# BuTTerK3ks/AA-RMVSNet

Measured on AMD Instinct MI355X. Metric: depth-hypotheses/sec (ref-views x H x W x D / s), higher is better.
Workload: dtype fp32-class split-fp16 (3 products: cells, deconvs, omega conv on f16 MFMA, lo*lo dropped, fp32 accumulate; fp32 elsewhere); 1 GPU; dtu_eval_1600x1184_n7_d512; ref_views_per_gpu=1, views=7, H=1184, W=1600, D=512, global_batch=1, parallelism=ref-view shard x1

## Files before the change

### aa-rmvsnet_amd/csrc/warp_cost.hip

```cpp
#include <hip/hip_runtime.h>

#include <cfloat>
#include <climits>
#include <cstdlib>
#include <cstring>

#include "device_common.h"

namespace aarmvs {

__device__ __forceinline__ void sample_pos(const float* __restrict__ m, float depth, float x,
                                           float y, int H, int W, float& ix, float& iy) {
  float p[3];
#pragma unroll
  for (int k = 0; k < 3; ++k) {
    const float rx = __fadd_rn(__fadd_rn(__fmul_rn(m[4 * k + 0], x), __fmul_rn(m[4 * k + 1], y)),
                               m[4 * k + 2]);
    p[k] = __fadd_rn(__fmul_rn(rx, depth), m[4 * k + 3]);
  }
  float z = p[2];
  if (z == 0.0f) z = __fadd_rn(z, 1e-4f);
  const float px = __fdiv_rn(p[0], z), py = __fdiv_rn(p[1], z);
  const float gx = __fsub_rn(__fdiv_rn(px, (float)(W - 1) * 0.5f), 1.0f);
  const float gy = __fsub_rn(__fdiv_rn(py, (float)(H - 1) * 0.5f), 1.0f);
// ... 677 lines not shown

typedef _Float16 half8 __attribute__((ext_vector_type(8)));
typedef _Float16 half4 __attribute__((ext_vector_type(4)));
typedef _Float16 half2_t __attribute__((ext_vector_type(2)));
typedef float float2_t __attribute__((ext_vector_type(2)));
typedef float floatx4 __attribute__((ext_vector_type(4)));
typedef float floatx16 __attribute__((ext_vector_type(16)));

typedef __attribute__((address_space(3))) void* lds_void_ptr;
__device__ __forceinline__ void dma16(__amdgpu_buffer_rsrc_t r, float* wave_dst, uint32_t off,
                                      uint32_t soff = 0) {
  __builtin_amdgcn_raw_ptr_buffer_load_lds(r, (lds_void_ptr)wave_dst, 16, off, soff, 0, 0);
}
__device__ __forceinline__ uint32_t split_pair(float a, float b, uint32_t& lo_bits) {
  const uint32_t hb = __builtin_bit_cast(uint32_t, __builtin_convertvector((float2_t){a, b}, half2_t));
  float la, lb;
  asm("v_fma_mix_f32 %0, %1, -1.0, %2 op_sel_hi:[1,0,0]" : "=v"(la) : "v"(hb), "v"(a));
  asm("v_fma_mix_f32 %0, %1, -1.0, %2 op_sel:[1,0,0] op_sel_hi:[1,0,0]" : "=v"(lb) : "v"(hb), "v"(b));
  lo_bits = __builtin_bit_cast(uint32_t, __builtin_convertvector((float2_t){la, lb}, half2_t));
  return hb;
}
__device__ __forceinline__ void dma_wait() {
  __builtin_amdgcn_s_waitcnt(0x0F70);
}


constexpr int kMTileH = 16;
template <int TW>
struct OmegaTile {
  static constexpr int NT = kMTileH * TW;
  static constexpr int OUTH = kMTileH - 2, OUTW = TW - 2;
  static constexpr int BOXPX = 2 * NT;
  static int tiles(int H, int W) { return ((W + OUTW - 1) / OUTW) * ((H + OUTH - 1) / OUTH); }
  __device__ static int tiles_d(int H, int W) { return ((W + OUTW - 1) / OUTW) * ((H + OUTH - 1) / OUTH); }
};
#ifndef AARMVS_OMEGA_TW
#define AARMVS_OMEGA_TW 16
#endif
constexpr int kOmegaTW = AARMVS_OMEGA_TW;

template <int CTRL, int ROWS>
__device__ __forceinline__ double dpp_f64_u(double v) {
  const long long b = __double_as_longlong(v);
  const int lo = __builtin_amdgcn_mov_dpp((int)(b & 0xffffffffll), CTRL, ROWS, 0xF, false);
  const int hi = __builtin_amdgcn_mov_dpp((int)(b >> 32), CTRL, ROWS, 0xF, false);
  return __longlong_as_double(((long long)hi << 32) | (unsigned)lo);
}
__device__ __forceinline__ void wave_sum2_d(double& u, double& w) {
  u += dpp_f64_u<0xB1, 0xF>(u);
  w += dpp_f64_u<0xB1, 0xF>(w);
  u += dpp_f64_u<0x4E, 0xF>(u);
  w += dpp_f64_u<0x4E, 0xF>(w);
  u += dpp_f64_u<0x141, 0xF>(u);
  w += dpp_f64_u<0x141, 0xF>(w);
  u += dpp_f64_u<0x140, 0xF>(u);
  w += dpp_f64_u<0x140, 0xF>(w);
  u += dpp_f64_u<0x142, 0xA>(u);
  w += dpp_f64_u<0x142, 0xA>(w);
  u += dpp_f64_u<0x143, 0xC>(u);
  w += dpp_f64_u<0x143, 0xC>(w);
  auto rl = [](double v) {
    const long long b = __double_as_longlong(v);
    const int lo = __builtin_amdgcn_readlane((int)(b & 0xffffffffll), 63);
    const int hi = __builtin_amdgcn_readlane((int)(b >> 32), 63);
    return __longlong_as_double(((long long)hi << 32) | (unsigned)lo);
  };
  u = rl(u);
  w = rl(w);
}

struct OmegaPos {
  int tile, ty, tx, v, kp;
};
template <int NW>
__device__ __forceinline__ void omega_block_sum(const double (*ws)[2], double& s0, double& s1) {
  s0 = 0.0;
  s1 = 0.0;
  for (int w = 0; w < NW; ++w) {
    s0 += ws[w][0];
    s1 += ws[w][1];
  }
}

template <int ABL, int TW, bool BAL, typename PA>
__device__ __forceinline__ void omega_item(PA& a, const float* __restrict__ P,
                                           const float* __restrict__ Rel,
                                           const unsigned* __restrict__ xbound, const OmegaPos ip,
                                           double (*wsum)[OmegaTile<TW>::NT / 64][2], int par,
                                           bool has_prev, const OmegaPos pv) {
  using T = OmegaTile<TW>;
  constexpr int kMThreads = T::NT, kMBoxPx = T::BOXPX, kMOutH = T::OUTH, kMOutW = T::OUTW;
  constexpr int NB = (2 * kMBoxPx + kMThreads - 1) / kMThreads;
  static_assert(TW == 16 || TW == 32, "the row sums shift by DPP along one haloed row");
  constexpr int kRefFl = (kMBoxPx + 1) * 8;
  constexpr int YFL = kRefFl + 2 * kMThreads * 4;
  static_assert(2 * kMThreads * 4 <= YFL, "the row-sum images fit in the box space");
  __shared__ __attribute__((aligned(16))) float smem[YFL];
  float* const box = smem;
  float4* const zms = reinterpret_cast<float4*>(smem);
  float4* const zps = zms + kMThreads;
  __shared__ int red[kMThreads / 64][4];
  int tid;
  asm volatile("v_mov_b32 %0, %1" : "=v"(tid) : "v"((int)threadIdx.x));
  const int lane = tid & 63, wave = tid >> 6;
  const int b = blockIdx.z;
  const int H = a.H, W = a.W, HW = H * W, nsrc = a.nsrc;
  const int v = ip.v, kp = ip.kp;
  const int y0 = ip.ty * kMOutH, x0 = ip.tx * kMOutW;
  const int hy = tid / TW, hx = tid % TW;
  const int gy = y0 - 1 + hy, gx = x0 - 1 + hx;
  const bool in_img = gy >= 0 && gy < H && gx >= 0 && gx < W;
  const bool interior = in_img && hy >= 1 && hy <= kMOutH && hx >= 1 && hx <= kMOutW;
  float* const rimg = smem + kRefFl;

  const float dep = a.dvals[b * a.D + a.d_next + kp];
  const float* __restrict__ m = Rel + 12 * (v * a.B + b);
  const uint32_t fbytes = (uint32_t)((size_t)kC * HW * 4);
  const uint32_t cbytes = (uint32_t)HW * 32u;
  const __amdgpu_buffer_rsrc_t rref = uniform_rsrc(a.ref + (size_t)b * kC * HW, fbytes);
  const __amdgpu_buffer_rsrc_t rsrc = uniform_rsrc(a.src[v] + (size_t)b * kC * HW, fbytes);
  TapF tf{};
  int lx = INT_MAX, ly = INT_MAX, bhx = INT_MIN, bhy = INT_MIN;
  if (in_img) {
    if constexpr ((ABL & 16) != 0) {
      tf.xf = (float)gx + 0.25f * dep * 1e-3f;
      tf.yf = (float)gy;
      tf.wt[0] = tf.wt[1] = tf.wt[2] = tf.wt[3] = 0.25f;
      tf.xf = floorf(tf.xf);
    } else {
      tf = tap_f(m, dep, gx, gy, H, W);
    }
    box_extend(tf, H, W, lx, ly, bhx, bhy);
  }
  const Box bx = box_reduce<kMThreads / 64>(lx, ly, bhx, bhy, red);
  if (tid < 8) box[kMBoxPx * 8 + tid] = 0.f;
  if (has_prev && tid == 0) {
    double s0, s1;
    omega_block_sum<kMThreads / 64>(wsum[par ^ 1], s0, s1);
    if (!(ABL & 64)) part_put(a, pv.kp, b, pv.v, pv.tile, s0, s1);
  }
  const bool lds = bx.nx * bx.ny <= min(kMBoxPx, a.box_cap);
  const uint32_t zp = lds ? (uint32_t)kMBoxPx : fbytes / 32u;
  TapP tp = tap_p4(tf, in_img, H, W, lds, bx, zp);
  const int items = lds ? bx.nx * bx.ny * 2 : 0;
  const uint32_t mg = box_magic(bx.nx);
  uint32_t boff[NB];
#pragma unroll
  for (int j = 0; j < NB; ++j) {
    const int i = tid + j * kMThreads, p = i >> 1, r = box_row(p, bx.nx, mg);
    const uint32_t gp = __umul24((uint32_t)(bx.y0 + r), (uint32_t)W) + (uint32_t)bx.x0 +
                        ((uint32_t)p - __umul24((uint32_t)r, (uint32_t)bx.nx));
    boff[j] = gp * 32u + 16u * (uint32_t)img_half((uint32_t)p, i & 1);
  }
  const uint32_t rpix = in_img ? (uint32_t)(gy * W + gx) * 32u : fbytes;
  const int wave_s = __builtin_amdgcn_readfirstlane(wave);
  auto stage = [&](int c) {
    const uint32_t cb = (uint32_t)c * cbytes;
#pragma unroll
    for (int j = 0; j < NB; ++j)
      if (!(ABL & 2) && tid + j * kMThreads < items)
        dma16(rsrc, box + (j * kMThreads + wave_s * 64) * 4, boff[j], cb);
    if (!(ABL & 8)) {
      dma16(rref, rimg + (wave_s * 64) * 4, rpix, cb);
      dma16(rref, rimg + (kMThreads + wave_s * 64) * 4, rpix + 16u, cb);
    }
  };
  int e = 0;
  {
    const float bound = __uint_as_float(*xbound);
    if (bound > 0.0f) {
      const int k = ilogbf(bound);
      e = k >= 134 ? 120 : (k < -100 ? -114 : k - 14);
      e += e & 1;
    }
  }
  const float dsc = ldexpf(1.0f, -(e / 2));
#pragma unroll
  for (int k = 0; k < 4; ++k) tp.wt[k] = __fmul_rn(tp.wt[k], dsc);
  const float* __restrict__ w0t = P + a.off_ow0t;
  const half8* __restrict__ owm = reinterpret_cast<const half8*>(P + a.off_owm);
  floatx16 acc0, acc1;
  if constexpr ((ABL & 1) != 0) {
#pragma unroll
    for (int r = 0; r < 16; ++r) acc0[r] = acc1[r] = 0.f;
  }
  float o4[4] = {0.f, 0.f, 0.f, 0.f};

  stage(0);
  dma_wait();
  __syncthreads();
#pragma unroll 1
  for (int c = 0; c < 4; ++c) {
    const float* const bx_c = box;
    float4 g0, g1;
    if (ABL & 4) {
      g0 = g1 = make_float4(tp.wt[0], tp.wt[1], tp.wt[2], tp.wt[3]);
    } else if (lds) {
      g0 = bil4(img_ld(bx_c, tp.pix[0], 0), img_ld(bx_c, tp.pix[1], 0), img_ld(bx_c, tp.pix[2], 0),
                img_ld(bx_c, tp.pix[3], 0), tp);
      g1 = bil4(img_ld(bx_c, tp.pix[0], 1), img_ld(bx_c, tp.pix[1], 1), img_ld(bx_c, tp.pix[2], 1),
                img_ld(bx_c, tp.pix[3], 1), tp);
    } else {
      g0 = bil4(ld_c8(rsrc, tp.pix[0], 2 * c, HW), ld_c8(rsrc, tp.pix[1], 2 * c, HW),
                ld_c8(rsrc, tp.pix[2], 2 * c, HW), ld_c8(rsrc, tp.pix[3], 2 * c, HW), tp);
      g1 = bil4(ld_c8(rsrc, tp.pix[0], 2 * c + 1, HW), ld_c8(rsrc, tp.pix[1], 2 * c + 1, HW),
                ld_c8(rsrc, tp.pix[2], 2 * c + 1, HW), ld_c8(rsrc, tp.pix[3], 2 * c + 1, HW), tp);
    }
    const float4 rf0 = *reinterpret_cast<const float4*>(rimg + tid * 4);
    const float4 rf1 = *reinterpret_cast<const float4*>(rimg + (kMThreads + tid) * 4);
    auto dsq = [&](float g, float r) {
      const float dd = __fmaf_rn(r, -dsc, g);
      return __fmul_rn(dd, dd);
    };
    const float sq[8] = {dsq(g0.x, rf0.x), dsq(g0.y, rf0.y), dsq(g0.z, rf0.z), dsq(g0.w, rf0.w),
                         dsq(g1.x, rf1.x), dsq(g1.y, rf1.y), dsq(g1.z, rf1.z), dsq(g1.w, rf1.w)};
    half8 Bd, Bl, Bl2;
    if constexpr ((ABL & 128) == 0) {
      Bd = owm[(c * 3 + 0) * 64 + lane];
      Bl = owm[(c * 3 + 1) * 64 + lane];
      Bl2 = owm[(c * 3 + 2) * 64 + lane];
    }
    __syncthreads();
    if (c < 3) stage(c + 1);
    {
      const float* wt = w0t + (4 * kC + 8 * c) * 4;
#pragma unroll
      for (int j = 0; j < 8; ++j)
#pragma unroll
        for (int co = 0; co < 4; ++co) o4[co] = fmaf(sq[j], wt[j * 4 + co], o4[co]);
    }
    uint32_t hw[4], lw[4];
#pragma unroll
    for (int i = 0; i < 4; ++i) hw[i] = split_pair(sq[2 * i], sq[2 * i + 1], lw[i]);
#pragma unroll
    for (int i = 0; i < 4; ++i) {
      const auto r = __builtin_amdgcn_permlane32_swap(hw[i], lw[i], false, false);
      hw[i] = r[0];
      lw[i] = r[1];
    }
    if (BAL && (c & 1)) {
#pragma unroll
      for (int i = 0; i < 4; ++i) {
        hw[i] ^= 0x80008000u;
        lw[i] ^= 0x80008000u;
      }
    }
    if (BAL && c > 0) {
#pragma unroll
      for (int r = 0; r < 16; ++r) {
        acc0[r] = -acc0[r];
        acc1[r] = -acc1[r];
      }
    }
    const half8 A0 = __builtin_bit_cast(half8, u32x4{hw[0], hw[1], hw[2], hw[3]});
    const half8 A1 = __builtin_bit_cast(half8, u32x4{lw[0], lw[1], lw[2], lw[3]});
    if constexpr ((ABL & 128) != 0) {
      Bd = A1;
      Bl = A0;
      Bl2 = A1;
    }
    if (!(ABL & 1)) {
      if (c == 0) {
        const floatx16 z = {};
        acc0 = __builtin_amdgcn_mfma_f32_32x32x16_f16(Bd, A0, z, 0, 0, 0);
        acc1 = __builtin_amdgcn_mfma_f32_32x32x16_f16(Bd, A1, z, 0, 0, 0);
      } else {
        acc0 = __builtin_amdgcn_mfma_f32_32x32x16_f16(Bd, A0, acc0, 0, 0, 0);
        acc1 = __builtin_amdgcn_mfma_f32_32x32x16_f16(Bd, A1, acc1, 0, 0, 0);
      }
      acc0 = __builtin_amdgcn_mfma_f32_32x32x16_f16(Bl, A0, acc0, 0, 0, 0);
      acc1 = __builtin_amdgcn_mfma_f32_32x32x16_f16(Bl, A1, acc1, 0, 0, 0);
      acc0 = __builtin_amdgcn_mfma_f32_32x32x16_f16(Bl2, A0, acc0, 0, 0, 0);
      acc1 = __builtin_amdgcn_mfma_f32_32x32x16_f16(Bl2, A1, acc1, 0, 0, 0);
    } else {
      acc0[0] += (float)A0[0] + (float)Bd[1];
      acc1[0] += (float)A1[0] + (float)Bl[1];
    }
    if (c < 3) {
      dma_wait();
      __syncthreads();
    }
  }
  static constexpr int kShr = TW == 16 ? 0x111 : 0x138, kShl = TW == 16 ? 0x101 : 0x130;
  auto shr1 = [](float x) {
    return __int_as_float(__builtin_amdgcn_update_dpp(0, __float_as_int(x), kShr, 0xF, 0xF, true));
  };
  auto shl1 = [](float x) {
    return __int_as_float(__builtin_amdgcn_update_dpp(0, __float_as_int(x), kShl, 0xF, 0xF, true));
  };
  float zmr[4], zpr[4], z0[4];
#pragma unroll
  for (int co = 0; co < 4; ++co) {
    const float r0 = (shr1(acc0[co]) + acc0[4 + co]) + shl1(acc0[8 + co]);
    const float r1 = (shr1(acc1[co]) + acc1[4 + co]) + shl1(acc1[8 + co]);
    const auto zz = __builtin_amdgcn_permlane32_swap(__float_as_uint(r0), __float_as_uint(r1), false, false);
    zmr[co] = __uint_as_float(zz[0]);
    zpr[co] = __uint_as_float(zz[1]);
    const auto t35 = __builtin_amdgcn_permlane32_swap(__float_as_uint(acc0[12 + co]),
                                                      __float_as_uint(acc1[12 + co]), false, false);
    z0[co] = shr1(__uint_as_float(t35[0])) + shl1(__uint_as_float(t35[1]));
  }
  if constexpr ((ABL & 32) == 0) {
    zms[tid] = make_float4(zmr[0], zmr[1], zmr[2], zmr[3]);
    zps[tid] = make_float4(zpr[0], zpr[1], zpr[2], zpr[3]);
  }
  __syncthreads();
  double ps = 0.0, pss = 0.0;
  if (interior) {
    float g4[4];
    if constexpr ((ABL & 32) != 0) {
#pragma unroll
      for (int co = 0; co < 4; ++co) g4[co] = (zmr[co] + z0[co]) + zpr[co];
    } else {
      const float4 up = zms[tid - TW], dn = zps[tid + TW];
      g4[0] = (up.x + z0[0]) + dn.x;
      g4[1] = (up.y + z0[1]) + dn.y;
      g4[2] = (up.z + z0[2]) + dn.z;
      g4[3] = (up.w + z0[3]) + dn.w;
    }
    if (BAL) {
#pragma unroll
      for (int co = 0; co < 4; ++co) g4[co] = -g4[co];
    }
    const float pe = ldexpf(1.0f, e);
    const float isc = P[a.off_owm_scale] * pe;
    const float* __restrict__ b0 = P + a.off_ob0;
    float4 out;
    out.x = fmaf(g4[0], isc, o4[0] * pe) + b0[0];
    out.y = fmaf(g4[1], isc, o4[1] * pe) + b0[1];
    out.z = fmaf(g4[2], isc, o4[2] * pe) + b0[2];
    out.w = fmaf(g4[3], isc, o4[3] * pe) + b0[3];
    a.t1_next[kp * a.t1_kstride + ((size_t)b * nsrc + v) * HW + gy * W + gx] = out;
    ps = ((double)out.x + (double)out.y) + ((double)out.z + (double)out.w);
    pss = ((double)out.x * out.x + (double)out.y * out.y) + ((double)out.z * out.z + (double)out.w * out.w);
  }
  wave_sum2_d(ps, pss);
  if (lane == 0) {
    wsum[par][wave][0] = ps;
    wsum[par][wave][1] = pss;
  }
}

#ifndef AARMVS_OMEGA_WAVES
#define AARMVS_OMEGA_WAVES 4
#endif
template <int ABL = 0, int TW = kOmegaTW, bool BAL = false>
__global__ void __launch_bounds__(OmegaTile<TW>::NT) __attribute__((amdgpu_waves_per_eu(AARMVS_OMEGA_WAVES)))
omega_mfma_kernel(PipeArgs a, const float* __restrict__ P, const float* __restrict__ Rel,
                  const unsigned* __restrict__ xbound) {
  if (blockDim.x != OmegaTile<TW>::NT) return;
  const int ipb = a.omega_ipb > 1 ? a.omega_ipb : 1;
  const int npl = a.npl, nsrc = a.nsrc;
  const int tiles_x = (a.W + OmegaTile<TW>::OUTW - 1) / OmegaTile<TW>::OUTW;
  const int total = OmegaTile<TW>::tiles_d(a.H, a.W) * nsrc * npl;
  const int seq0 = xcd_tile(blockIdx.x, gridDim.x) * ipb;
  OmegaPos ip;
  ip.tile = seq0 / (nsrc * npl);
  {
    const int vk = seq0 - ip.tile * (nsrc * npl);
    ip.v = vk / npl;
    ip.kp = vk - ip.v * npl;
    ip.ty = ip.tile / tiles_x;
    ip.tx = ip.tile - ip.ty * tiles_x;
  }
  constexpr int NW = OmegaTile<TW>::NT / 64;
  __shared__ double wsum[2][NW][2];
  OmegaPos pv = ip;
  int it = 0;
#pragma unroll 1
  for (; it < ipb; ++it) {
    if (seq0 + it >= total) break;
    if (it) {
      pv = ip;
      if (++ip.kp == npl) {
        ip.kp = 0;
        if (++ip.v == nsrc) {
          ip.v = 0;
          ++ip.tile;
          if (++ip.tx == tiles_x) {
            ip.tx = 0;
            ++ip.ty;
          }
        }
      }
    }
    uint32_t z;
    asm volatile("s_mov_b32 %0, 0" : "=s"(z));
    typedef const __attribute__((address_space(4))) PipeArgs KPipeArgs;
    KPipeArgs& ka = *(KPipeArgs*)((const __attribute__((address_space(4))) char*)&a + z);
    omega_item<ABL, TW, BAL>(ka, P, Rel, xbound, ip, wsum, it & 1, it > 0, pv);
  }
  if (it > 0) {
    __syncthreads();
    if (threadIdx.x == 0) {
      double s0, s1;
      omega_block_sum<NW>(wsum[(it - 1) & 1], s0, s1);
      if (!(ABL & 64)) part_put(a, ip.kp, (int)blockIdx.z, ip.v, ip.tile, s0, s1);
    }
  }
}

template <int STAGE>
__global__ void __launch_bounds__(256) omega_stats_kernel(PipeArgs a,
                                                          const float* __restrict__ P) {
  __shared__ double red[2 * 4];
  __shared__ GnStat gs[2];
  const int v = blockIdx.y, b = blockIdx.z / a.npl, kp = blockIdx.z - b * a.npl;
  const int HW = a.H * a.W;
  double* const st = a.st_next + kp * a.st_kstride;
  if (threadIdx.x < STAGE)
    gs[threadIdx.x] = stat_read(st + st_index(b, v, threadIdx.x, a.nsrc), 4.0 * HW);
  __syncthreads();
  OmegaP o;
  load_omega(a, P, o);
  const float4* t1 = a.t1_next + kp * a.t1_kstride + ((size_t)b * a.nsrc + v) * HW;
  double part[2] = {0.0, 0.0};
  const int gstride = gridDim.x * blockDim.x;
  for (int p0 = blockIdx.x * blockDim.x + threadIdx.x; p0 < HW; p0 += 4 * gstride) {
    float4 qs[4];
#pragma unroll
    for (int u = 0; u < 4; ++u) {
      const int p = p0 + u * gstride;
      qs[u] = p < HW ? t1[p] : make_float4(0.f, 0.f, 0.f, 0.f);
    }
#pragma unroll
    for (int u = 0; u < 4; ++u) {
    if (p0 + u * gstride >= HW) break;
    const float4 q = qs[u];
    const float t[4] = {q.x, q.y, q.z, q.w};
    float aa[4], t2[4];
    gn_relu4(t, gs[0], o.g0w, o.g0b, true, aa);
    conv1x1_4(aa, o.w1, o.b1, t2);
    float r[4];
    if constexpr (STAGE == 1) {
#pragma unroll
      for (int c = 0; c < 4; ++c) r[c] = t2[c];
    } else {
      float bb[4];
      gn_relu4(t2, gs[1], o.g1w, o.g1b, true, bb);
      conv1x1_4(bb, o.w2, o.b2, r);
    }
    part[0] += ((double)r[0] + (double)r[1]) + ((double)r[2] + (double)r[3]);
    part[1] += ((double)r[0] * r[0] + (double)r[1] * r[1]) + ((double)r[2] * r[2] + (double)r[3] * r[3]);
    }
  }
  block_sum_d<2>(part, red);
  if (threadIdx.x == 0) part_put(a, kp, b, v, blockIdx.x, part[0], part[1]);
}

__global__ void __launch_bounds__(256) stat_reduce_kernel(PipeArgs a, int stage) {
  __shared__ double red[2][256];
  const int g = blockIdx.x, v = g % a.nsrc, b = (g / a.nsrc) % a.B, kp = g / (a.nsrc * a.B);
  const double* pp = a.part + 2 * (size_t)g * a.part_n;
  double s = 0.0, ss = 0.0;
  for (int i = threadIdx.x; i < a.part_n; i += 256) {
    s += pp[2 * i];
    ss += pp[2 * i + 1];
  }
  red[0][threadIdx.x] = s;
  red[1][threadIdx.x] = ss;
  __syncthreads();
  for (int o = 128; o > 0; o >>= 1) {
    if (threadIdx.x < o) {
      red[0][threadIdx.x] += red[0][threadIdx.x + o];
      red[1][threadIdx.x] += red[1][threadIdx.x + o];
    }
    __syncthreads();
  }
  if (threadIdx.x == 0) {
    double* st = a.st_next + kp * a.st_kstride + st_index(b, v, stage, a.nsrc);
    st[0] = red[0][0];
    st[1] = red[1][0];
  }
}

static PipeArgs pipe_args(const CostArgs& ca, const SweepGeom& g, const Workspace& ws) {
  const ParamLayout& L = param_layout();
  PipeArgs a{};
  a.ref = ca.ref;
  for (int v = 0; v < AARMVS_MAX_SRC; ++v) a.src[v] = v < g.nsrc ? ca.src[v] : nullptr;
  a.rel = ca.rel;
  a.dvals = ca.depth_values;
  a.D = g.D;
  a.params = ca.params;
  a.x = ws.x;
  a.B = g.B;
  a.H = g.H;
  a.W = g.W;
  a.nsrc = g.nsrc;
  a.box_cap = INT_MAX;
  a.npl = 1;
  a.omega_k = 0;
  a.off_ow0 = L.pk_off[P_OW0];
  a.off_ow0t = L.ow0t_off;
  a.off_owb_scale = L.owb_scale_off;
  a.off_owm = L.owm_off;
  a.off_owm_scale = L.owb_scale_off;
  a.off_ob0 = L.pk_off[P_OB0];
  a.off_og0w = L.pk_off[P_OG0W];
  a.off_og0b = L.pk_off[P_OG0B];
  a.off_ow1 = L.pk_off[P_OW1];
  a.off_ob1 = L.pk_off[P_OB1];
  a.off_og1w = L.pk_off[P_OG1W];
  a.off_og1b = L.pk_off[P_OG1B];
  a.off_ow2 = L.pk_off[P_OW2];
  a.off_ob2 = L.pk_off[P_OB2];
  a.off_og2w = L.pk_off[P_OG2W];
  a.off_og2b = L.pk_off[P_OG2B];
  a.off_owo = L.pk_off[P_OWO];
  a.off_obo = L.pk_off[P_OBO];
  return a;
}

static int pipe_box_cap() {
  const char* s = std::getenv("AARMVS_PIPE_BOX_CAP");
  return (s && *s) ? std::max(4, std::atoi(s)) : INT_MAX;
}

static int omega_ipb(int items, int cu_count) {
  const char* s = std::getenv("AARMVS_OMEGA_IPB");
  if (s && *s) return std::max(1, std::min(8, std::atoi(s)));
  int ipb = 8;
  while (ipb > 1 && (items + ipb - 1) / ipb < 8 * std::max(1, cu_count)) ipb >>= 1;
  return ipb;
}

constexpr int kCostXPlanes = 2;
static int cost_x_planes() {
  const char* s = std::getenv("AARMVS_COST_X_PLANES");
  const int v = (s && *s) ? std::atoi(s) : kCostXPlanes;
  return v >= 4 ? 4 : v >= 2 ? 2 : 1;
}

static PipeArgs pipe_args_c8(const CostArgs& ca, const SweepGeom& g, const Workspace& ws) {
  PipeArgs a = pipe_args(ca, g, ws);
  a.ref = ws.feat8[0];
  for (int v = 0; v < g.nsrc; ++v) a.src[v] = ws.feat8[1 + v];
  a.box_cap = pipe_box_cap();
  return a;
}

static void group_strides(PipeArgs& a, const Workspace& ws, int n) {
  a.npl = n;
  a.t1_kstride = ws.t1_plane;
  a.st_kstride = ws.omega_stats_bytes / sizeof(double);
  a.x_kstride = ws.x_plane;
}

hipError_t launch_cost_x_group(const CostArgs& ca, const SweepGeom& g, const Workspace& ws, int d0,
                               int n, float* x0, float* omega_out, int omega_k, hipStream_t s) {
  PipeArgs a = pipe_args_c8(ca, g, ws);
  group_strides(a, ws, n);
  a.d_prev = d0;
  a.d_next = -1;
  a.x = x0;
  a.t1_prev = reinterpret_cast<const float4*>(ws.t1);
  a.st_prev = ws.omega_stats;
  a.omega_out = omega_out;
  a.omega_k = omega_out ? omega_k : -1;
  const int ntiles = ((g.W + kTileW - 1) / kTileW) * ((g.H + kXRows - 1) / kXRows);
  const int pp = cost_x_planes();
  const dim3 grid(ntiles * ((n + pp - 1) / pp), g.B), block(2 * kXRows * kTileW);
  ProfScope ps(s, K_COST_X);
  if (pp == 4)
    hipLaunchKernelGGL((cost_x_planes_kernel<kXRows, 4>), grid, block, 0, s, a, a.params, a.rel);
  else if (pp == 2)
    hipLaunchKernelGGL((cost_x_planes_kernel<kXRows, 2>), grid, block, 0, s, a, a.params, a.rel);
  else
    hipLaunchKernelGGL(cost_x_kernel<2>, grid, block, 0, s, a, a.params, a.rel);
  return hipGetLastError();
}

hipError_t launch_omega_group(const CostArgs& ca, const SweepGeom& g, const Workspace& ws, int d0,
                              int n, hipStream_t s, bool balanced) {
  PipeArgs a = pipe_args_c8(ca, g, ws);
  group_strides(a, ws, n);
  a.d_prev = -1;
  a.d_next = d0;
  a.t1_next = reinterpret_cast<float4*>(ws.t1);
  a.st_next = ws.omega_stats;
  a.part = ws.omega_part;
  hipError_t e;
  const int nred = n * g.B * g.nsrc;
  if ((e = hipMemsetAsync(ws.omega_stats, 0, (size_t)n * ws.omega_stats_bytes, s)) != hipSuccess)
    return e;
  {
    const int ntiles = OmegaTile<kOmegaTW>::tiles(g.H, g.W);
    ProfScope ps(s, K_OMEGA_CONV);
    a.part_n = ntiles;
    a.omega_ipb = omega_ipb(ntiles * g.nsrc * n * g.B, g.cu_count);
    const int nblk = (ntiles * g.nsrc * n + a.omega_ipb - 1) / a.omega_ipb;
    if (balanced)
      hipLaunchKernelGGL((omega_mfma_kernel<0, kOmegaTW, true>), dim3(nblk, 1, g.B),
                         dim3(OmegaTile<kOmegaTW>::NT), 0, s, a, a.params, a.rel, ws.xbound);
    else
      hipLaunchKernelGGL((omega_mfma_kernel<0, kOmegaTW>), dim3(nblk, 1, g.B),
                         dim3(OmegaTile<kOmegaTW>::NT), 0, s, a, a.params, a.rel, ws.xbound);
    if ((e = hipGetLastError()) != hipSuccess) return e;
  }
  {
    ProfScope ps(s, K_STAT_REDUCE);
    hipLaunchKernelGGL(stat_reduce_kernel, dim3(nred), dim3(256), 0, s, a, 0);
  }
  if ((e = hipGetLastError()) != hipSuccess) return e;
  const int HW = g.H * g.W;
  const int pblk =
      std::max(1, std::min((HW + 1023) / 1024, 8 * g.cu_count / std::max(1, g.B * g.nsrc) + 1));
  a.part_n = pblk;
  {
    ProfScope ps(s, K_OMEGA1);
    hipLaunchKernelGGL(omega_stats_kernel<1>, dim3(pblk, g.nsrc, g.B * n), dim3(256), 0, s, a,
                       a.params);
  }
  if ((e = hipGetLastError()) != hipSuccess) return e;
  {
    ProfScope ps(s, K_STAT_REDUCE);
    hipLaunchKernelGGL(stat_reduce_kernel, dim3(nred), dim3(256), 0, s, a, 1);
  }
  if ((e = hipGetLastError()) != hipSuccess) return e;
  {
    ProfScope ps(s, K_OMEGA2);
    hipLaunchKernelGGL(omega_stats_kernel<2>, dim3(pblk, g.nsrc, g.B * n), dim3(256), 0, s, a,
                       a.params);
  }
  if ((e = hipGetLastError()) != hipSuccess) return e;
  {
    ProfScope ps(s, K_STAT_REDUCE);
    hipLaunchKernelGGL(stat_reduce_kernel, dim3(nred), dim3(256), 0, s, a, 2);
  }
  return hipGetLastError();
}

__global__ void __launch_bounds__(256) nchw_to_c8_kernel(const float* __restrict__ src,
                                                         float* __restrict__ dst, int HW,
                                                         unsigned* __restrict__ xbound) {
  __shared__ float t[kC][65];
  __shared__ float wmax[4];
  const int b = blockIdx.y, p0 = blockIdx.x * 64;
  const float* s = src + (size_t)b * kC * HW;
  float4* d = reinterpret_cast<float4*>(dst + (size_t)b * kC * HW);
  const int px = threadIdx.x & 63;
  float mx = 0.f;
#pragma unroll
  for (int j = 0; j < 8; ++j) {
    const int c = (threadIdx.x >> 6) + 4 * j;
    const float v = p0 + px < HW ? s[(size_t)c * HW + p0 + px] : 0.f;
    t[c][px] = v;
    const float av = fabsf(v);
    mx = (av > mx || av != av) ? av : mx;
  }
  if (xbound) {
#pragma unroll
    for (int o = 32; o > 0; o >>= 1) {
      const float q = __shfl_xor(mx, o, 64);
      mx = (q > mx || q != q) ? q : mx;
    }
    if ((threadIdx.x & 63) == 0) wmax[threadIdx.x >> 6] = mx;
  }
  __syncthreads();
  if (xbound && threadIdx.x == 0) {
    float m = 0.f;
    for (int w = 0; w < 4; ++w) m = (wmax[w] > m || wmax[w] != wmax[w]) ? wmax[w] : m;
    const float bound = 8.0f * m * m;
    const unsigned bits = __float_as_uint(bound != bound ? INFINITY : bound);
    if (bits > __hip_atomic_load(xbound, __ATOMIC_RELAXED, __HIP_MEMORY_SCOPE_AGENT))
      atomicMax(xbound, bits);
  }
#pragma unroll
  for (int j = 0; j < 2; ++j) {
    const int idx = threadIdx.x + 256 * j, ch = idx >> 7, q = (idx & 127) >> 1, h = idx & 1;
    const int c0 = 8 * ch + 4 * h;
    if (p0 + q < HW)
      d[((size_t)ch * HW + p0 + q) * 2 + h] =
          make_float4(t[c0][q], t[c0 + 1][q], t[c0 + 2][q], t[c0 + 3][q]);
  }
}
// ... 897 lines not shown
```

Measured before the change: 1.230 billion depth-hypotheses/s.

## Process two depth planes per omega item sharing one staged source box

The omega MFMA kernel can now handle a pair of adjacent depth planes in one item. Both planes' taps are folded into one shared LDS source box, so the staged box, the reference image reads and the weight fragments are loaded once and serve two planes of MFMA accumulation. If the combined box does not fit in LDS, the kernel falls back to single-plane items. This is meant to cut the repeated DMA staging and synchronisation per plane, at the cost of more live registers (waves_per_eu is lowered to 3) and more complex control flow. It is enabled by default when there are multiple planes per group and the unbalanced path is in use.

Result: faster. 1.260 billion depth-hypotheses/s (median of 6 runs) (+2.5%).

```diff
diff --git a/aa-rmvsnet_amd/csrc/warp_cost.hip b/aa-rmvsnet_amd/csrc/warp_cost.hip
--- a/aa-rmvsnet_amd/csrc/warp_cost.hip
+++ b/aa-rmvsnet_amd/csrc/warp_cost.hip
@@ -783,24 +783,31 @@
   }
 }
 
-template <int ABL, int TW, bool BAL, typename PA>
-__device__ __forceinline__ void omega_item(PA& a, const float* __restrict__ P,
+template <int TW>
+struct OmegaLds {
+  using T = OmegaTile<TW>;
+  static constexpr int kRefFl = (T::BOXPX + 1) * 8;
+  static constexpr int YFL = kRefFl + 2 * T::NT * 4;
+  static_assert(2 * 2 * T::NT * 4 <= YFL, "two planes' row-sum images fit in the box space");
+};
+
+template <int ABL, int TW, bool BAL, int PP, int KPP, typename PA>
+__device__ __forceinline__ bool omega_item(PA& a, const float* __restrict__ P,
                                            const float* __restrict__ Rel,
                                            const unsigned* __restrict__ xbound, const OmegaPos ip,
-                                           double (*wsum)[OmegaTile<TW>::NT / 64][2], int par,
-                                           bool has_prev, const OmegaPos pv) {
+                                           double (*wsum)[KPP][OmegaTile<TW>::NT / 64][2], int par,
+                                           int nprev, const OmegaPos pv, float* const smem,
+                                           int (*red)[4]) {
   using T = OmegaTile<TW>;
   constexpr int kMThreads = T::NT, kMBoxPx = T::BOXPX, kMOutH = T::OUTH, kMOutW = T::OUTW;
   constexpr int NB = (2 * kMBoxPx + kMThreads - 1) / kMThreads;
   static_assert(TW == 16 || TW == 32, "the row sums shift by DPP along one haloed row");
-  constexpr int kRefFl = (kMBoxPx + 1) * 8;
-  constexpr int YFL = kRefFl + 2 * kMThreads * 4;
-  static_assert(2 * kMThreads * 4 <= YFL, "the row-sum images fit in the box space");
-  __shared__ __attribute__((aligned(16))) float smem[YFL];
+  static_assert(PP == 1 || PP == 2, "one plane or a plane pair per item");
+  static_assert(PP <= KPP, "the wave sums hold KPP planes per item");
+  constexpr int kRefFl = OmegaLds<TW>::kRefFl;
   float* const box = smem;
   float4* const zms = reinterpret_cast<float4*>(smem);
   float4* const zps = zms + kMThreads;
-  __shared__ int red[kMThreads / 64][4];
   int tid;
   asm volatile("v_mov_b32 %0, %1" : "=v"(tid) : "v"((int)threadIdx.x));
   const int lane = tid & 63, wave = tid >> 6;
@@ -814,35 +821,51 @@
   const bool interior = in_img && hy >= 1 && hy <= kMOutH && hx >= 1 && hx <= kMOutW;
   float* const rimg = smem + kRefFl;
 
-  const float dep = a.dvals[b * a.D + a.d_next + kp];
   const float* __restrict__ m = Rel + 12 * (v * a.B + b);
   const uint32_t fbytes = (uint32_t)((size_t)kC * HW * 4);
   const uint32_t cbytes = (uint32_t)HW * 32u;
   const __amdgpu_buffer_rsrc_t rref = uniform_rsrc(a.ref + (size_t)b * kC * HW, fbytes);
   const __amdgpu_buffer_rsrc_t rsrc = uniform_rsrc(a.src[v] + (size_t)b * kC * HW, fbytes);
-  TapF tf{};
+  TapF tf[PP] = {};
   int lx = INT_MAX, ly = INT_MAX, bhx = INT_MIN, bhy = INT_MIN;
-  if (in_img) {
-    if constexpr ((ABL & 16) != 0) {
-      tf.xf = (float)gx + 0.25f * dep * 1e-3f;
-      tf.yf = (float)gy;
-      tf.wt[0] = tf.wt[1] = tf.wt[2] = tf.wt[3] = 0.25f;
-      tf.xf = floorf(tf.xf);
-    } else {
-      tf = tap_f(m, dep, gx, gy, H, W);
-    }
-    box_extend(tf, H, W, lx, ly, bhx, bhy);
+#pragma unroll
+  for (int q = 0; q < PP; ++q) {
+    const float dep = a.dvals[b * a.D + a.d_next + kp + q];
+    if (in_img) {
+      if constexpr ((ABL & 16) != 0) {
+        tf[q].xf = (float)gx + 0.25f * dep * 1e-3f;
+        tf[q].yf = (float)gy;
+        tf[q].wt[0] = tf[q].wt[1] = tf[q].wt[2] = tf[q].wt[3] = 0.25f;
+        tf[q].xf = floorf(tf[q].xf);
+      } else {
+        tf[q] = tap_f(m, dep, gx, gy, H, W);
+      }
+      box_extend(tf[q], H, W, lx, ly, bhx, bhy);
+    }
   }
   const Box bx = box_reduce<kMThreads / 64>(lx, ly, bhx, bhy, red);
-  if (tid < 8) box[kMBoxPx * 8 + tid] = 0.f;
-  if (has_prev && tid == 0) {
-    double s0, s1;
-    omega_block_sum<kMThreads / 64>(wsum[par ^ 1], s0, s1);
-    if (!(ABL & 64)) part_put(a, pv.kp, b, pv.v, pv.tile, s0, s1);
+  if constexpr (PP == 1) {
+    if (tid < 8) box[kMBoxPx * 8 + tid] = 0.f;
+  }
+  if (nprev && tid == 0) {
+#pragma unroll
+    for (int q = 0; q < KPP; ++q) {
+      if (q < nprev) {
+        double s0, s1;
+        omega_block_sum<kMThreads / 64>(wsum[par ^ 1][q], s0, s1);
+        if (!(ABL & 64)) part_put(a, pv.kp + q, b, pv.v, pv.tile, s0, s1);
+      }
+    }
   }
   const bool lds = bx.nx * bx.ny <= min(kMBoxPx, a.box_cap);
+  if constexpr (PP > 1) {
+    if (!lds) return false;
+    if (tid < 8) box[kMBoxPx * 8 + tid] = 0.f;
+  }
   const uint32_t zp = lds ? (uint32_t)kMBoxPx : fbytes / 32u;
-  TapP tp = tap_p4(tf, in_img, H, W, lds, bx, zp);
+  TapP tp[PP];
+#pragma unroll
+  for (int q = 0; q < PP; ++q) tp[q] = tap_p4(tf[q], in_img, H, W, lds, bx, zp);
   const int items = lds ? bx.nx * bx.ny * 2 : 0;
   const uint32_t mg = box_magic(bx.nx);
   uint32_t boff[NB];
@@ -877,15 +900,19 @@
   }
   const float dsc = ldexpf(1.0f, -(e / 2));
 #pragma unroll
-  for (int k = 0; k < 4; ++k) tp.wt[k] = __fmul_rn(tp.wt[k], dsc);
+  for (int q = 0; q < PP; ++q)
+#pragma unroll
+    for (int k = 0; k < 4; ++k) tp[q].wt[k] = __fmul_rn(tp[q].wt[k], dsc);
   const float* __restrict__ w0t = P + a.off_ow0t;
   const half8* __restrict__ owm = reinterpret_cast<const half8*>(P + a.off_owm);
-  floatx16 acc0, acc1;
+  floatx16 acc0[PP], acc1[PP];
   if constexpr ((ABL & 1) != 0) {
 #pragma unroll
-    for (int r = 0; r < 16; ++r) acc0[r] = acc1[r] = 0.f;
-  }
-  float o4[4] = {0.f, 0.f, 0.f, 0.f};
+    for (int q = 0; q < PP; ++q)
+#pragma unroll
+      for (int r = 0; r < 16; ++r) acc0[q][r] = acc1[q][r] = 0.f;
+  }
+  float o4[PP][4] = {};
 
   stage(0);
   dma_wait();
@@ -893,90 +920,120 @@
 #pragma unroll 1
   for (int c = 0; c < 4; ++c) {
     const float* const bx_c = box;
-    float4 g0, g1;
-    if (ABL & 4) {
-      g0 = g1 = make_float4(tp.wt[0], tp.wt[1], tp.wt[2], tp.wt[3]);
-    } else if (lds) {
-      g0 = bil4(img_ld(bx_c, tp.pix[0], 0), img_ld(bx_c, tp.pix[1], 0), img_ld(bx_c, tp.pix[2], 0),
-                img_ld(bx_c, tp.pix[3], 0), tp);
-      g1 = bil4(img_ld(bx_c, tp.pix[0], 1), img_ld(bx_c, tp.pix[1], 1), img_ld(bx_c, tp.pix[2], 1),
-                img_ld(bx_c, tp.pix[3], 1), tp);
-    } else {
-      g0 = bil4(ld_c8(rsrc, tp.pix[0], 2 * c, HW), ld_c8(rsrc, tp.pix[1], 2 * c, HW),
-                ld_c8(rsrc, tp.pix[2], 2 * c, HW), ld_c8(rsrc, tp.pix[3], 2 * c, HW), tp);
-      g1 = bil4(ld_c8(rsrc, tp.pix[0], 2 * c + 1, HW), ld_c8(rsrc, tp.pix[1], 2 * c + 1, HW),
-                ld_c8(rsrc, tp.pix[2], 2 * c + 1, HW), ld_c8(rsrc, tp.pix[3], 2 * c + 1, HW), tp);
-    }
-    const float4 rf0 = *reinterpret_cast<const float4*>(rimg + tid * 4);
-    const float4 rf1 = *reinterpret_cast<const float4*>(rimg + (kMThreads + tid) * 4);
+    float4 rf0, rf1;
+    auto ref_read = [&]() {
+      rf0 = *reinterpret_cast<const float4*>(rimg + tid * 4);
+      rf1 = *reinterpret_cast<const float4*>(rimg + (kMThreads + tid) * 4);
+    };
+    if constexpr (PP > 1) ref_read();
     auto dsq = [&](float g, float r) {
       const float dd = __fmaf_rn(r, -dsc, g);
       return __fmul_rn(dd, dd);
     };
-    const float sq[8] = {dsq(g0.x, rf0.x), dsq(g0.y, rf0.y), dsq(g0.z, rf0.z), dsq(g0.w, rf0.w),
-                         dsq(g1.x, rf1.x), dsq(g1.y, rf1.y), dsq(g1.z, rf1.z), dsq(g1.w, rf1.w)};
+    auto sample = [&](int q, float (&sq)[8]) {
+      const TapP& t = tp[q];
+      float4 g0, g1;
+      if (ABL & 4) {
+        g0 = g1 = make_float4(t.wt[0], t.wt[1], t.wt[2], t.wt[3]);
+      } else if (PP > 1 || lds) {
+        g0 = bil4(img_ld(bx_c, t.pix[0], 0), img_ld(bx_c, t.pix[1], 0), img_ld(bx_c, t.pix[2], 0),
+                  img_ld(bx_c, t.pix[3], 0), t);
+        g1 = bil4(img_ld(bx_c, t.pix[0], 1), img_ld(bx_c, t.pix[1], 1), img_ld(bx_c, t.pix[2], 1),
+                  img_ld(bx_c, t.pix[3], 1), t);
+      } else {
+        g0 = bil4(ld_c8(rsrc, t.pix[0], 2 * c, HW), ld_c8(rsrc, t.pix[1], 2 * c, HW),
+                  ld_c8(rsrc, t.pix[2], 2 * c, HW), ld_c8(rsrc, t.pix[3], 2 * c, HW), t);
+        g1 = bil4(ld_c8(rsrc, t.pix[0], 2 * c + 1, HW), ld_c8(rsrc, t.pix[1], 2 * c + 1, HW),
+                  ld_c8(rsrc, t.pix[2], 2 * c + 1, HW), ld_c8(rsrc, t.pix[3], 2 * c + 1, HW), t);
+      }
+      if constexpr (PP == 1) ref_read();
+      sq[0] = dsq(g0.x, rf0.x);
+      sq[1] = dsq(g0.y, rf0.y);
+      sq[2] = dsq(g0.z, rf0.z);
+      sq[3] = dsq(g0.w, rf0.w);
+      sq[4] = dsq(g1.x, rf1.x);
+      sq[5] = dsq(g1.y, rf1.y);
+      sq[6] = dsq(g1.z, rf1.z);
+      sq[7] = dsq(g1.w, rf1.w);
+    };
     half8 Bd, Bl, Bl2;
-    if constexpr ((ABL & 128) == 0) {
-      Bd = owm[(c * 3 + 0) * 64 + lane];
-      Bl = owm[(c * 3 + 1) * 64 + lane];
-      Bl2 = owm[(c * 3 + 2) * 64 + lane];
-    }
+    auto accumulate = [&](int q, const float (&sq)[8]) {
+      {
+        const float* wt = w0t + (4 * kC + 8 * c) * 4;
+#pragma unroll
+        for (int j = 0; j < 8; ++j)
+#pragma unroll
+          for (int co = 0; co < 4; ++co) o4[q][co] = fmaf(sq[j], wt[j * 4 + co], o4[q][co]);
+      }
+      uint32_t hw[4], lw[4];
+#pragma unroll
+      for (int i = 0; i < 4; ++i) hw[i] = split_pair(sq[2 * i], sq[2 * i + 1], lw[i]);
+#pragma unroll
+      for (int i = 0; i < 4; ++i) {
+        const auto r = __builtin_amdgcn_permlane32_swap(hw[i], lw[i], false, false);
+        hw[i] = r[0];
+        lw[i] = r[1];
+      }
+      if (BAL && (c & 1)) {
+#pragma unroll
+        for (int i = 0; i < 4; ++i) {
+          hw[i] ^= 0x80008000u;
+          lw[i] ^= 0x80008000u;
+        }
+      }
+      if (BAL && c > 0) {
+#pragma unroll
+        for (int r = 0; r < 16; ++r) {
+          acc0[q][r] = -acc0[q][r];
+          acc1[q][r] = -acc1[q][r];
+        }
+      }
+      const half8 A0 = __builtin_bit_cast(half8, u32x4{hw[0], hw[1], hw[2], hw[3]});
+      const half8 A1 = __builtin_bit_cast(half8, u32x4{lw[0], lw[1], lw[2], lw[3]});
+      if constexpr ((ABL & 128) != 0) {
+        Bd = A1;
+        Bl = A0;
+        Bl2 = A1;
+      }
+      if (!(ABL & 1)) {
+        if (c == 0) {
+          const floatx16 z = {};
+          acc0[q] = __builtin_amdgcn_mfma_f32_32x32x16_f16(Bd, A0, z, 0, 0, 0);
+          acc1[q] = __builtin_amdgcn_mfma_f32_32x32x16_f16(Bd, A1, z, 0, 0, 0);
+        } else {
+          acc0[q] = __builtin_amdgcn_mfma_f32_32x32x16_f16(Bd, A0, acc0[q], 0, 0, 0);
+          acc1[q] = __builtin_amdgcn_mfma_f32_32x32x16_f16(Bd, A1, acc1[q], 0, 0, 0);
+        }
+        acc0[q] = __builtin_amdgcn_mfma_f32_32x32x16_f16(Bl, A0, acc0[q], 0, 0, 0);
+        acc1[q] = __builtin_amdgcn_mfma_f32_32x32x16_f16(Bl, A1, acc1[q], 0, 0, 0);
+        acc0[q] = __builtin_amdgcn_mfma_f32_32x32x16_f16(Bl2, A0, acc0[q], 0, 0, 0);
+        acc1[q] = __builtin_amdgcn_mfma_f32_32x32x16_f16(Bl2, A1, acc1[q], 0, 0, 0);
+      } else {
+        acc0[q][0] += (float)A0[0] + (float)Bd[1];
+        acc1[q][0] += (float)A1[0] + (float)Bl[1];
+      }
+    };
+    auto fragments = [&]() {
+      if constexpr ((ABL & 128) == 0) {
+        Bd = owm[(c * 3 + 0) * 64 + lane];
+        Bl = owm[(c * 3 + 1) * 64 + lane];
+        Bl2 = owm[(c * 3 + 2) * 64 + lane];
+      }
+    };
+    float sq[PP][8];
+#pragma unroll
+    for (int q = 0; q < PP; ++q) {
+      sample(q, sq[q]);
+      if constexpr (PP > 1) {
+#pragma unroll
+        for (int j = 0; j < 8; ++j) asm volatile("" : "+v"(sq[q][j]));
+      }
+    }
+    fragments();
     __syncthreads();
     if (c < 3) stage(c + 1);
-    {
-      const float* wt = w0t + (4 * kC + 8 * c) * 4;
-#pragma unroll
-      for (int j = 0; j < 8; ++j)
-#pragma unroll
-        for (int co = 0; co < 4; ++co) o4[co] = fmaf(sq[j], wt[j * 4 + co], o4[co]);
-    }
-    uint32_t hw[4], lw[4];
-#pragma unroll
-    for (int i = 0; i < 4; ++i) hw[i] = split_pair(sq[2 * i], sq[2 * i + 1], lw[i]);
-#pragma unroll
-    for (int i = 0; i < 4; ++i) {
-      const auto r = __builtin_amdgcn_permlane32_swap(hw[i], lw[i], false, false);
-      hw[i] = r[0];
-      lw[i] = r[1];
-    }
-    if (BAL && (c & 1)) {
-#pragma unroll
-      for (int i = 0; i < 4; ++i) {
-        hw[i] ^= 0x80008000u;
-        lw[i] ^= 0x80008000u;
-      }
-    }
-    if (BAL && c > 0) {
-#pragma unroll
-      for (int r = 0; r < 16; ++r) {
-        acc0[r] = -acc0[r];
-        acc1[r] = -acc1[r];
-      }
-    }
-    const half8 A0 = __builtin_bit_cast(half8, u32x4{hw[0], hw[1], hw[2], hw[3]});
-    const half8 A1 = __builtin_bit_cast(half8, u32x4{lw[0], lw[1], lw[2], lw[3]});
-    if constexpr ((ABL & 128) != 0) {
-      Bd = A1;
-      Bl = A0;
-      Bl2 = A1;
-    }
-    if (!(ABL & 1)) {
-      if (c == 0) {
-        const floatx16 z = {};
-        acc0 = __builtin_amdgcn_mfma_f32_32x32x16_f16(Bd, A0, z, 0, 0, 0);
-        acc1 = __builtin_amdgcn_mfma_f32_32x32x16_f16(Bd, A1, z, 0, 0, 0);
-      } else {
-        acc0 = __builtin_amdgcn_mfma_f32_32x32x16_f16(Bd, A0, acc0, 0, 0, 0);
-        acc1 = __builtin_amdgcn_mfma_f32_32x32x16_f16(Bd, A1, acc1, 0, 0, 0);
-      }
-      acc0 = __builtin_amdgcn_mfma_f32_32x32x16_f16(Bl, A0, acc0, 0, 0, 0);
-      acc1 = __builtin_amdgcn_mfma_f32_32x32x16_f16(Bl, A1, acc1, 0, 0, 0);
-      acc0 = __builtin_amdgcn_mfma_f32_32x32x16_f16(Bl2, A0, acc0, 0, 0, 0);
-      acc1 = __builtin_amdgcn_mfma_f32_32x32x16_f16(Bl2, A1, acc1, 0, 0, 0);
-    } else {
-      acc0[0] += (float)A0[0] + (float)Bd[1];
-      acc1[0] += (float)A1[0] + (float)Bl[1];
-    }
+#pragma unroll
+    for (int q = 0; q < PP; ++q) accumulate(q, sq[q]);
     if (c < 3) {
       dma_wait();
       __syncthreads();
@@ -989,67 +1046,77 @@
   auto shl1 = [](float x) {
     return __int_as_float(__builtin_amdgcn_update_dpp(0, __float_as_int(x), kShl, 0xF, 0xF, true));
   };
-  float zmr[4], zpr[4], z0[4];
-#pragma unroll
-  for (int co = 0; co < 4; ++co) {
-    const float r0 = (shr1(acc0[co]) + acc0[4 + co]) + shl1(acc0[8 + co]);
-    const float r1 = (shr1(acc1[co]) + acc1[4 + co]) + shl1(acc1[8 + co]);
-    const auto zz = __builtin_amdgcn_permlane32_swap(__float_as_uint(r0), __float_as_uint(r1), false, false);
-    zmr[co] = __uint_as_float(zz[0]);
-    zpr[co] = __uint_as_float(zz[1]);
-    const auto t35 = __builtin_amdgcn_permlane32_swap(__float_as_uint(acc0[12 + co]),
-                                                      __float_as_uint(acc1[12 + co]), false, false);
-    z0[co] = shr1(__uint_as_float(t35[0])) + shl1(__uint_as_float(t35[1]));
-  }
-  if constexpr ((ABL & 32) == 0) {
-    zms[tid] = make_float4(zmr[0], zmr[1], zmr[2], zmr[3]);
-    zps[tid] = make_float4(zpr[0], zpr[1], zpr[2], zpr[3]);
+  float zmr[PP][4], zpr[PP][4], z0[PP][4];
+#pragma unroll
+  for (int q = 0; q < PP; ++q) {
+#pragma unroll
+    for (int co = 0; co < 4; ++co) {
+      const float r0 = (shr1(acc0[q][co]) + acc0[q][4 + co]) + shl1(acc0[q][8 + co]);
+      const float r1 = (shr1(acc1[q][co]) + acc1[q][4 + co]) + shl1(acc1[q][8 + co]);
+      const auto zz = __builtin_amdgcn_permlane32_swap(__float_as_uint(r0), __float_as_uint(r1), false, false);
+      zmr[q][co] = __uint_as_float(zz[0]);
+      zpr[q][co] = __uint_as_float(zz[1]);
+      const auto t35 = __builtin_amdgcn_permlane32_swap(__float_as_uint(acc0[q][12 + co]),
+                                                        __float_as_uint(acc1[q][12 + co]), false, false);
+      z0[q][co] = shr1(__uint_as_float(t35[0])) + shl1(__uint_as_float(t35[1]));
+    }
+    if constexpr ((ABL & 32) == 0) {
+      zms[2 * q * kMThreads + tid] = make_float4(zmr[q][0], zmr[q][1], zmr[q][2], zmr[q][3]);
+      zps[2 * q * kMThreads + tid] = make_float4(zpr[q][0], zpr[q][1], zpr[q][2], zpr[q][3]);
+    }
   }
   __syncthreads();
-  double ps = 0.0, pss = 0.0;
-  if (interior) {
-    float g4[4];
-    if constexpr ((ABL & 32) != 0) {
-#pragma unroll
-      for (int co = 0; co < 4; ++co) g4[co] = (zmr[co] + z0[co]) + zpr[co];
-    } else {
-      const float4 up = zms[tid - TW], dn = zps[tid + TW];
-      g4[0] = (up.x + z0[0]) + dn.x;
-      g4[1] = (up.y + z0[1]) + dn.y;
-      g4[2] = (up.z + z0[2]) + dn.z;
-      g4[3] = (up.w + z0[3]) + dn.w;
-    }
-    if (BAL) {
-#pragma unroll
-      for (int co = 0; co < 4; ++co) g4[co] = -g4[co];
-    }
-    const float pe = ldexpf(1.0f, e);
-    const float isc = P[a.off_owm_scale] * pe;
-    const float* __restrict__ b0 = P + a.off_ob0;
-    float4 out;
-    out.x = fmaf(g4[0], isc, o4[0] * pe) + b0[0];
-    out.y = fmaf(g4[1], isc, o4[1] * pe) + b0[1];
-    out.z = fmaf(g4[2], isc, o4[2] * pe) + b0[2];
-    out.w = fmaf(g4[3], isc, o4[3] * pe) + b0[3];
-    a.t1_next[kp * a.t1_kstride + ((size_t)b * nsrc + v) * HW + gy * W + gx] = out;
-    ps = ((double)out.x + (double)out.y) + ((double)out.z + (double)out.w);
-    pss = ((double)out.x * out.x + (double)out.y * out.y) + ((double)out.z * out.z + (double)out.w * out.w);
-  }
-  wave_sum2_d(ps, pss);
-  if (lane == 0) {
-    wsum[par][wave][0] = ps;
-    wsum[par][wave][1] = pss;
-  }
+#pragma unroll
+  for (int q = 0; q < PP; ++q) {
+    double ps = 0.0, pss = 0.0;
+    if (interior) {
+      float g4[4];
+      if constexpr ((ABL & 32) != 0) {
+#pragma unroll
+        for (int co = 0; co < 4; ++co) g4[co] = (zmr[q][co] + z0[q][co]) + zpr[q][co];
+      } else {
+        const float4 up = zms[2 * q * kMThreads + tid - TW], dn = zps[2 * q * kMThreads + tid + TW];
+        g4[0] = (up.x + z0[q][0]) + dn.x;
+        g4[1] = (up.y + z0[q][1]) + dn.y;
+        g4[2] = (up.z + z0[q][2]) + dn.z;
+        g4[3] = (up.w + z0[q][3]) + dn.w;
+      }
+      if (BAL) {
+#pragma unroll
+        for (int co = 0; co < 4; ++co) g4[co] = -g4[co];
+      }
+      const float pe = ldexpf(1.0f, e);
+      const float isc = P[a.off_owm_scale] * pe;
+      const float* __restrict__ b0 = P + a.off_ob0;
+      float4 out;
+      out.x = fmaf(g4[0], isc, o4[q][0] * pe) + b0[0];
+      out.y = fmaf(g4[1], isc, o4[q][1] * pe) + b0[1];
+      out.z = fmaf(g4[2], isc, o4[q][2] * pe) + b0[2];
+      out.w = fmaf(g4[3], isc, o4[q][3] * pe) + b0[3];
+      a.t1_next[(kp + q) * a.t1_kstride + ((size_t)b * nsrc + v) * HW + gy * W + gx] = out;
+      ps = ((double)out.x + (double)out.y) + ((double)out.z + (double)out.w);
+      pss = ((double)out.x * out.x + (double)out.y * out.y) + ((double)out.z * out.z + (double)out.w * out.w);
+    }
+    wave_sum2_d(ps, pss);
+    if (lane == 0) {
+      wsum[par][q][wave][0] = ps;
+      wsum[par][q][wave][1] = pss;
+    }
+  }
+  return true;
 }
 
 #ifndef AARMVS_OMEGA_WAVES
 #define AARMVS_OMEGA_WAVES 4
 #endif
-template <int ABL = 0, int TW = kOmegaTW, bool BAL = false>
-__global__ void __launch_bounds__(OmegaTile<TW>::NT) __attribute__((amdgpu_waves_per_eu(AARMVS_OMEGA_WAVES)))
+template <int ABL = 0, int TW = kOmegaTW, bool BAL = false, int KPP = 1>
+__global__ void __launch_bounds__(OmegaTile<TW>::NT)
+__attribute__((amdgpu_waves_per_eu(KPP > 1 ? 3 : AARMVS_OMEGA_WAVES)))
 omega_mfma_kernel(PipeArgs a, const float* __restrict__ P, const float* __restrict__ Rel,
                   const unsigned* __restrict__ xbound) {
   if (blockDim.x != OmegaTile<TW>::NT) return;
+  __shared__ __attribute__((aligned(16))) float smem[OmegaLds<TW>::YFL];
+  __shared__ int red[KPP][OmegaTile<TW>::NT / 64][4];
   const int ipb = a.omega_ipb > 1 ? a.omega_ipb : 1;
   const int npl = a.npl, nsrc = a.nsrc;
   const int tiles_x = (a.W + OmegaTile<TW>::OUTW - 1) / OmegaTile<TW>::OUTW;
@@ -1065,15 +1132,69 @@
     ip.tx = ip.tile - ip.ty * tiles_x;
   }
   constexpr int NW = OmegaTile<TW>::NT / 64;
-  __shared__ double wsum[2][NW][2];
+  __shared__ double wsum[2][KPP][NW][2];
   OmegaPos pv = ip;
-  int it = 0;
+  if constexpr (KPP == 1) {
+    int it = 0;
 #pragma unroll 1
-  for (; it < ipb; ++it) {
-    if (seq0 + it >= total) break;
-    if (it) {
+    for (; it < ipb; ++it) {
+      if (seq0 + it >= total) break;
+      if (it) {
+        pv = ip;
+        if (++ip.kp == npl) {
+          ip.kp = 0;
+          if (++ip.v == nsrc) {
+            ip.v = 0;
+            ++ip.tile;
+            if (++ip.tx == tiles_x) {
+              ip.tx = 0;
+              ++ip.ty;
+            }
+          }
+        }
+      }
+      uint32_t z;
+      asm volatile("s_mov_b32 %0, 0" : "=s"(z));
+      typedef const __attribute__((address_space(4))) PipeArgs KPipeArgs;
+      KPipeArgs& ka = *(KPipeArgs*)((const __attribute__((address_space(4))) char*)&a + z);
+      omega_item<ABL, TW, BAL, 1, 1>(ka, P, Rel, xbound, ip, wsum, it & 1, it > 0, pv, smem, red[0]);
+    }
+    if (it > 0) {
+      __syncthreads();
+      if (threadIdx.x == 0) {
+        double s0, s1;
+        omega_block_sum<NW>(wsum[(it - 1) & 1][0], s0, s1);
+        if (!(ABL & 64)) part_put(a, ip.kp, (int)blockIdx.z, ip.v, ip.tile, s0, s1);
+      }
+    }
+  } else {
+    int it = 0, np = 0, par = 0, singles = 0;
+#pragma unroll 1
+    while (it < ipb && seq0 + it < total) {
+      uint32_t z;
+      asm volatile("s_mov_b32 %0, 0" : "=s"(z));
+      typedef const __attribute__((address_space(4))) PipeArgs KPipeArgs;
+      KPipeArgs& ka = *(KPipeArgs*)((const __attribute__((address_space(4))) char*)&a + z);
+      int done = 0;
+      if (singles == 0 && it + 1 < ipb && seq0 + it + 1 < total && ip.kp + 1 < npl) {
+        if (omega_item<ABL, TW, BAL, 2, KPP>(ka, P, Rel, xbound, ip, wsum, par, np, pv, smem, red[1]))
+          done = 2;
+        else {
+          np = 0;
+          singles = 2;
+        }
+      }
+      if (done == 0) {
+        omega_item<ABL, TW, BAL, 1, KPP>(ka, P, Rel, xbound, ip, wsum, par, np, pv, smem, red[0]);
+        done = 1;
+        if (singles) --singles;
+      }
       pv = ip;
-      if (++ip.kp == npl) {
+      np = done;
+      par ^= 1;
+      it += done;
+      ip.kp += done;
+      if (ip.kp == npl) {
         ip.kp = 0;
         if (++ip.v == nsrc) {
           ip.v = 0;
@@ -1085,18 +1206,18 @@
         }
       }
     }
-    uint32_t z;
-    asm volatile("s_mov_b32 %0, 0" : "=s"(z));
-    typedef const __attribute__((address_space(4))) PipeArgs KPipeArgs;
-    KPipeArgs& ka = *(KPipeArgs*)((const __attribute__((address_space(4))) char*)&a + z);
-    omega_item<ABL, TW, BAL>(ka, P, Rel, xbound, ip, wsum, it & 1, it > 0, pv);
-  }
-  if (it > 0) {
-    __syncthreads();
-    if (threadIdx.x == 0) {
-      double s0, s1;
-      omega_block_sum<NW>(wsum[(it - 1) & 1], s0, s1);
-      if (!(ABL & 64)) part_put(a, ip.kp, (int)blockIdx.z, ip.v, ip.tile, s0, s1);
+    if (np > 0) {
+      __syncthreads();
+      if (threadIdx.x == 0) {
+#pragma unroll
+        for (int q = 0; q < KPP; ++q) {
+          if (q < np) {
+            double s0, s1;
+            omega_block_sum<NW>(wsum[par ^ 1][q], s0, s1);
+            if (!(ABL & 64)) part_put(a, pv.kp + q, (int)blockIdx.z, pv.v, pv.tile, s0, s1);
+          }
+        }
+      }
     }
   }
 }
@@ -1226,6 +1347,13 @@
   return ipb;
 }
 
+constexpr int kOmegaPlanes = 2;
+static int omega_planes() {
+  const char* s = std::getenv("AARMVS_OMEGA_PLANES");
+  const int v = (s && *s) ? std::atoi(s) : kOmegaPlanes;
+  return v >= 2 ? 2 : 1;
+}
+
 constexpr int kCostXPlanes = 2;
 static int cost_x_planes() {
   const char* s = std::getenv("AARMVS_COST_X_PLANES");
@@ -1293,6 +1421,9 @@
     const int nblk = (ntiles * g.nsrc * n + a.omega_ipb - 1) / a.omega_ipb;
     if (balanced)
       hipLaunchKernelGGL((omega_mfma_kernel<0, kOmegaTW, true>), dim3(nblk, 1, g.B),
+                         dim3(OmegaTile<kOmegaTW>::NT), 0, s, a, a.params, a.rel, ws.xbound);
+    else if (n > 1 && a.omega_ipb > 1 && omega_planes() == 2)
+      hipLaunchKernelGGL((omega_mfma_kernel<0, kOmegaTW, false, 2>), dim3(nblk, 1, g.B),
                          dim3(OmegaTile<kOmegaTW>::NT), 0, s, a, a.params, a.rel, ws.xbound);
     else
       hipLaunchKernelGGL((omega_mfma_kernel<0, kOmegaTW>), dim3(nblk, 1, g.B),
```
